# Lainshower/debiasing-multi-modal

Hardware: AMD Instinct MI355X
Metric: images/sec (embed+adapter step), CLIP-RN50 224px bs=1024 (higher is better)
Workload: dtype f32; 1 GPU; CLIP-RN50 224px encode_image + adapter(1024-128-1024) CE/SGD step, 1024 images/GPU, global batch 1024 (the metric's configuration, CLIP-RN50 224px bs=1024 on one GPU); global_batch=1024, batch_per_gpu=1024, parallelism=dp1, collective=none

## Files before the change

### debiasing-multi-modal_amd/csrc/bottleneck_chain.hip

```cpp
#include <stdlib.h>
#include "common.h"

namespace {

struct ChainP {
    const float* a; const float* a_absmax;
    const u16* w3; int w3_exp; const float* sc3; const float* b3;
    const float* res; float* x; float* xp; float* x_absmax;
    const u16* w1; int w1_exp; const float* sc1; const float* b1;
    float* y1; float* y1_absmax;
    int M, N;
    int Ho, Wo;
    const float* a2; const float* a2_absmax; const u16* wd; const float* ratio;
    const u16* w2; int w2_exp; const float* sc2; const float* b2;
    int H, W;
};

template <int RH>
__device__ __forceinline__ int swz(int row) { return RH == 32 ? ((row >> 2) & 3) : (RH == 64 ? ((row >> 1) & 7) : (row & 15)); }

constexpr int BM = 128;

template <int K, int P>
struct ChainGeo {
    static constexpr int BNS = K == 64 ? 64 : 32;
    static constexpr int SLROW = BNS + 4;
    static constexpr int R1_BYTES = BM * SLROW * 4 > 2 * BM * 64 * 2 ? BM * SLROW * 4 : 2 * BM * 64 * 2;
    static constexpr int W3_BYTES = BNS * K * 2;
    static constexpr int W1_BYTES = P * BNS * 2;
    static constexpr int LDS_BYTES = R1_BYTES + W3_BYTES + W1_BYTES;
};

template <int POOL>
__device__ __forceinline__ int row_pixel(const ChainP& p, int m) {
    if constexpr (!POOL) return m;
    const int mp = m >> 2, q = m & 3, wp2 = p.Wo >> 1, hwp = (p.Ho >> 1) * wp2;
    const int n = mp / hwp, rem = mp - n * hwp, hp = rem / wp2;
    return (n * p.Ho + 2 * hp + (q >> 1)) * p.Wo + 2 * (rem - hp * wp2) + (q & 1);
}

constexpr int C2_SROWS = 132, C2_PLANE = C2_SROWS * 32;
constexpr int C2_W2P = 104;
template <int K>
struct Conv2Geo {
    static constexpr int W2_OFF = 2 * C2_PLANE;
    static constexpr int GROUP_BYTES = (2 * C2_PLANE * 2 + K * C2_W2P * 2 + 255) / 256 * 256;
    static constexpr int NST = K == 64 ? 2 : 1;
    static constexpr int Z_OFF = NST * GROUP_BYTES;
    static constexpr int BYTES = Z_OFF + 256;
    static constexpr int STAGE_BYTES = BM * 68 * 4;
};
constexpr int cmax(int a, int b) { return a > b ? a : b; }

template <int K, int P, int POOL, int DUAL = 0, int CONV2 = 0>
__global__ __launch_bounds__(256, 2) void bottleneck_chain_kernel(const ChainP p) {
    static_assert(!DUAL || K == 64, "dual-source variant: layer-1 geometry (K = K2 = 64)");
    static_assert(!CONV2 || !POOL, "the conv2 phase walks pixels in standard order");
    static_assert(K == 64 || K == 128, "conv3 reduction depth: 64 (layer 1) or 128 (layer 2)");
    static_assert(P == 64 || P == 128, "conv1' width");
    using G = ChainGeo<K, P>;
    constexpr int BNS = G::BNS, SLROW = G::SLROW;
    constexpr int KS = K / 16, TN3 = BNS / 32, TN1 = P / 32;
    constexpr int LDS_TOTAL = cmax(G::LDS_BYTES + (DUAL ? BNS * 64 * 2 : 0), CONV2 ? cmax(Conv2Geo<K>::BYTES, Conv2Geo<K>::STAGE_BYTES) : 0);
    __shared__ __attribute__((aligned(256))) unsigned char lds_raw[LDS_TOTAL];
    u16* Ay = (u16*)lds_raw;
    float* slab = (float*)lds_raw;
    u16* W3b = (u16*)(lds_raw + G::R1_BYTES);
    u16* W1b = (u16*)(lds_raw + G::R1_BYTES + G::W3_BYTES);
    u16* Wdb = (u16*)(lds_raw + G::R1_BYTES + G::W3_BYTES + G::W1_BYTES);

    const int tid = threadIdx.x, lane = tid & 63, wave = tid >> 6;
    const int fr = lane & 31, fh = lane >> 5;
    const int m0 = xcd_remap(blockIdx.x, gridDim.x) * BM;
    const int NT = p.N / BNS;

    const int g0 = row_pixel<POOL>(p, m0);
    const long long Mll = p.M;
    const __amdgpu_buffer_rsrc_t rsA = desc(p.a, Mll * K * 4, (long long)g0 * K * 4);
    const __amdgpu_buffer_rsrc_t rsR = DUAL ? desc(p.a2, Mll * 64 * 4, (long long)g0 * 64 * 4)
                                            : desc(p.res, Mll * p.N * 4, (long long)g0 * p.N * 4);
    const __amdgpu_buffer_rsrc_t rsX = desc(p.x, POOL == 2 ? 0 : Mll * p.N * 4, (long long)g0 * p.N * 4);
    const __amdgpu_buffer_rsrc_t rsY = desc(p.y1, Mll * P * 4, (long long)g0 * P * 4);
    __amdgpu_buffer_rsrc_t rsXP = rsX;
    if constexpr (POOL) rsXP = desc(p.xp, (Mll >> 2) * p.N * 4, (long long)(m0 >> 2) * p.N * 4);

    unsigned gx[4], gy[4];
#pragma unroll
    for (int t = 0; t < 4; ++t) {
        const int m = m0 + wave * 32 + 8 * t + 4 * fh;
        const int dp = row_pixel<POOL>(p, m) - g0;
        gx[t] = m < p.M ? (unsigned)dp * (unsigned)(p.N * 4) + (unsigned)(fr * 4) : OOR;
        gy[t] = m < p.M ? (unsigned)dp * (unsigned)(P * 4) + (unsigned)(fr * 4) : OOR;
    }
    auto qpix = [&](int q) { return POOL ? (q >> 1) * p.Wo + (q & 1) : q; };

    constexpr int CPR3 = K / 8, RPP3 = 256 / CPR3, W3LD = BNS * CPR3 / 256;
    constexpr int CPR1 = BNS / 8, RPP1 = 256 / CPR1, W1LD = P * CPR1 / 256;
    static_assert(W3LD >= 1 && W1LD >= 1, "weight slabs smaller than one pass of the workgroup");
    const int wc3 = tid % CPR3, wr3 = tid / CPR3, wc1 = tid % CPR1, wr1 = tid / CPR1;
    u32x4 w3r[W3LD], w1r[W1LD], wdr[DUAL ? W3LD : 1];
    auto load_w = [&](int nt) {
#pragma unroll
        for (int j = 0; j < W3LD; ++j) {
            w3r[j] = *(const u32x4*)(p.w3 + (size_t)(nt * BNS + wr3 + RPP3 * j) * K + wc3 * 8);
            if constexpr (DUAL) wdr[j] = *(const u32x4*)(p.wd + (size_t)(nt * BNS + wr3 + RPP3 * j) * 64 + wc3 * 8);
        }
#pragma unroll
        for (int j = 0; j < W1LD; ++j)
            w1r[j] = *(const u32x4*)(p.w1 + (size_t)(wr1 + RPP1 * j) * p.N + nt * BNS + wc1 * 8);
    };
    auto store_w = [&]() {
#pragma unroll
        for (int j = 0; j < W3LD; ++j) {
            const int row = wr3 + RPP3 * j;
            *(u32x4*)(W3b + row * K + ((wc3 ^ swz<K>(row)) << 3)) = w3r[j];
            if constexpr (DUAL) *(u32x4*)(Wdb + row * 64 + ((wc3 ^ swz<64>(row)) << 3)) = wdr[j];
        }
// ... 44 lines not shown
        __syncthreads();
#pragma unroll
        for (int ks = 0; ks < 4; ++ks) {
            const int row = wave * 32 + fr;
            const int off = row * 64 + (((2 * ks + fh) ^ swz<64>(row)) << 3);
            dst[ks][0] = *(const u32x4*)(Ay + off);
            dst[ks][1] = *(const u32x4*)(Ay + BM * 64 + off);
        }
    };
    auto stage_pass = [&](const __amdgpu_buffer_rsrc_t& rs, int ldk, int k0, float sc, u32x4 (*dst)[2]) {
        f32x4 q[8];
        stage_issue(rs, ldk, k0, q);
        stage_finish(q, sc, dst);
    };
    f32x4 q2[(DUAL && CONV2) ? 8 : 1];
    if constexpr (DUAL && CONV2) stage_issue(rsR, 64, 0, q2);
    int s_a;
    if constexpr (!CONV2) {
        s_a = scale_exp(*p.a_absmax);
#pragma unroll
        for (int kp = 0; kp < K / 64; ++kp) stage_pass(rsA, K, kp * 64, pow2f(s_a), af + kp * 4);
    } else {
        using C2 = Conv2Geo<K>;
        constexpr int TN2 = K / 32, NG = (K / 32) * 3, W2LD = (K * 12 + 255) / 256;
        u16* Sp = (u16*)lds_raw;
        constexpr int NST = C2::NST, STH = C2::GROUP_BYTES / 2;
        constexpr int ZLH = C2::Z_OFF / 2;
        if (tid < 16) *(u32x4*)(lds_raw + C2::Z_OFF + tid * 16) = (u32x4){0u, 0u, 0u, 0u};
        const int s_y1 = scale_exp(*p.a_absmax);
        const float y1_sc = pow2f(s_y1);
        const int px0 = m0 - 1 - p.W > 0 ? m0 - 1 - p.W : 0;
        const __amdgpu_buffer_rsrc_t rsS = desc(p.a, Mll * K * 4, (long long)px0 * K * 4);
        const int lc = tid & 7, lr = tid >> 3;
        unsigned s_off[5];
#pragma unroll
        for (int i = 0; i < 5; ++i) {
            const int j = lr + 32 * i;
            s_off[i] = j < 130 ? (unsigned)((m0 - 1 + j - px0) * (K * 4)) + lc * 16u : OOR;
        }
        unsigned fmask = 0;
        {
            const int m = m0 + wave * 32 + fr;
            if (m < p.M) {
                const int hw = p.H * p.W, rem = m - (m / hw) * hw, ho = rem / p.W, wo = rem - ho * p.W;
#pragma unroll
                for (int kh = 0; kh < 3; ++kh)
#pragma unroll
                    for (int kw = 0; kw < 3; ++kw)
                        if (ho + kh - 1 >= 0 && ho + kh - 1 < p.H && wo + kw - 1 >= 0 && wo + kw - 1 < p.W) fmask |= 1u << (kh * 3 + kw);
            }
        }
        f32x4 sq[5];
        u32x4 w2q[W2LD];
        auto load_group = [&](int g) {
            const int sl = g / 3, kh = g - sl * 3;
            const unsigned delta = (unsigned)(((kh - 1) * p.W * K + sl * 32) * 4);
#pragma unroll
            for (int i = 0; i < 5; ++i)
                sq[i] = __builtin_bit_cast(f32x4, __builtin_amdgcn_raw_buffer_load_b128(rsS, s_off[i] == OOR ? OOR : s_off[i] + delta, 0, 0));
#pragma unroll
            for (int i = 0; i < W2LD; ++i) {
                const int idx = tid + 256 * i, row = idx / 12, c = idx - row * 12;
                w2q[i] = idx < K * 12 ? *(const u32x4*)(p.w2 + (size_t)row * (9 * K) + (size_t)g * 96 + c * 8) : (u32x4){0u, 0u, 0u, 0u};
            }
        };
        auto store_group = [&](int st) {
            u16* Sps = Sp + st * STH;
            u16* W2b = Sps + C2::W2_OFF;
#pragma unroll
            for (int i = 0; i < 5; ++i) {
                const int row = lr + 32 * i;
                if (row < 130) {
                    unsigned hp[2], lp[2];
#pragma unroll
                    for (int j = 0; j < 2; ++j) split2h_pair(sq[i][2 * j], sq[i][2 * j + 1], y1_sc, hp[j], lp[j]);
                    const int off = row * 32 + (((lc >> 1) ^ swz<32>(row)) << 3) + ((lc & 1) << 2);
                    *(u32x2*)(Sps + off) = (u32x2){hp[0], hp[1]};
                    *(u32x2*)(Sps + C2_PLANE + off) = (u32x2){lp[0], lp[1]};
                }
            }
#pragma unroll
            for (int i = 0; i < W2LD; ++i) {
                const int idx = tid + 256 * i, row = idx / 12, c = idx - row * 12;
                if (idx < K * 12) *(u32x4*)(W2b + row * C2_W2P + c * 8) = w2q[i];
            }
        };
        f32x16 acc2[TN2];
#pragma unroll
        for (int j = 0; j < TN2; ++j)
#pragma unroll
            for (int r = 0; r < 16; ++r) acc2[j][r] = 0.f;
        auto compute_group = [&](int g, int st) {
            const u16* Sps = Sp + st * STH;
            const u16* W2b = Sps + C2::W2_OFF;
            const int zl = ZLH - st * STH;
            const int kh = g % 3;
#pragma unroll
            for (int kw = 0; kw < 3; ++kw) {
                const bool ok = (fmask >> (kh * 3 + kw)) & 1u;
                const int row = wave * 32 + fr + kw;
#pragma unroll
                for (int ks = 0; ks < 2; ++ks) {
                    const int addr = row * 32 + (((2 * ks + fh) ^ swz<32>(row)) << 3);
                    const int a0 = ok ? addr : zl + (addr & 127), a1 = ok ? addr + C2_PLANE : zl + (addr & 127);
                    const u32x4 ah = *(const u32x4*)(Sps + a0), al = *(const u32x4*)(Sps + a1);
                    u32x4 wf[TN2];
#pragma unroll
                    for (int j = 0; j < TN2; ++j) wf[j] = *(const u32x4*)(W2b + (j * 32 + fr) * C2_W2P + kw * 32 + (2 * ks + fh) * 8);
#pragma unroll
                    for (int j = 0; j < TN2; ++j)
                        acc2[j] = __builtin_amdgcn_mfma_f32_32x32x16_f16(__builtin_bit_cast(f16x8, al), __builtin_bit_cast(f16x8, wf[j]), acc2[j], 0, 0, 0);
#pragma unroll
                    for (int j = 0; j < TN2; ++j)
                        acc2[j] = __builtin_amdgcn_mfma_f32_32x32x16_f16(__builtin_bit_cast(f16x8, ah), __builtin_bit_cast(f16x8, wf[j]), acc2[j], 0, 0, 0);
                }
            }
        };
        load_group(0);
        if constexpr (NST == 2) {
            store_group(0);
            __syncthreads();
            for (int g = 0; g < NG; ++g) {
                if (g + 1 < NG) load_group(g + 1);
                compute_group(g, g & 1);
                if (g + 1 < NG) store_group((g + 1) & 1);
                __syncthreads();
            }
        } else {
            for (int g = 0; g < NG; ++g) {
                store_group(0);
                __syncthreads();
                if (g + 1 < NG) load_group(g + 1);
                compute_group(g, 0);
                __syncthreads();
            }
        }
        const float c2_scale = pow2f(-s_y1 - p.w2_exp);
        float ymax = 0.f;
#pragma unroll
        for (int j = 0; j < TN2; ++j) {
            const float sv = p.sc2[j * 32 + fr] * c2_scale, bv = p.b2[j * 32 + fr];
#pragma unroll
            for (int r = 0; r < 16; ++r) {
                float v = fmaxf(fmaf(acc2[j][r], sv, bv), 0.f);
                if (gx[r >> 2] == OOR) v = 0.f;
                acc2[j][r] = v;
                ymax = fmaxf(ymax, v);
            }
        }
        s_a = scale_exp(wave_max(ymax));
        const float y2_sc = pow2f(s_a);
        float* St = (float*)lds_raw + wave * (32 * 68);
#pragma unroll
        for (int h = 0; h < K / 64; ++h) {
#pragma unroll
            for (int jj = 0; jj < 2; ++jj)
#pragma unroll
                for (int r = 0; r < 16; ++r) St[((r & 3) + 8 * (r >> 2) + 4 * fh) * 68 + jj * 32 + fr] = acc2[2 * h + jj][r];
#pragma unroll
            for (int ks = 0; ks < 4; ++ks) {
                const f32x4 x0 = *(const f32x4*)(St + fr * 68 + 16 * ks + 8 * fh), x1 = *(const f32x4*)(St + fr * 68 + 16 * ks + 8 * fh + 4);
                unsigned hh[4], ll[4];
                split2h_pair(x0[0], x0[1], y2_sc, hh[0], ll[0]); split2h_pair(x0[2], x0[3], y2_sc, hh[1], ll[1]);
                split2h_pair(x1[0], x1[1], y2_sc, hh[2], ll[2]); split2h_pair(x1[2], x1[3], y2_sc, hh[3], ll[3]);
// ... 29 lines not shown
        f32x16 acc3[TN3];
#pragma unroll
        for (int j = 0; j < TN3; ++j)
#pragma unroll
            for (int r = 0; r < 16; ++r) acc3[j][r] = 0.f;
        if constexpr (DUAL) {
#pragma unroll
            for (int ks = 0; ks < 4; ++ks) {
                u32x4 wf[TN3];
#pragma unroll
                for (int j = 0; j < TN3; ++j) {
                    const int row = j * 32 + fr;
                    wf[j] = *(const u32x4*)(Wdb + row * 64 + (((2 * ks + fh) ^ swz<64>(row)) << 3));
                }
#pragma unroll
                for (int pl = 1; pl >= 0; --pl)
#pragma unroll
                    for (int j = 0; j < TN3; ++j)
                        acc3[j] = __builtin_amdgcn_mfma_f32_32x32x16_f16(__builtin_bit_cast(f16x8, af2[ks][pl]),
                                                                         __builtin_bit_cast(f16x8, wf[j]), acc3[j], 0, 0, 0);
            }
#pragma unroll
            for (int j = 0; j < TN3; ++j) {
                const float rt = p.ratio[n0 + j * 32 + fr] * dual_dyn;
#pragma unroll
                for (int r = 0; r < 16; ++r) acc3[j][r] *= rt;
            }
        }
#pragma unroll
        for (int ks = 0; ks < KS; ++ks) {
            u32x4 wf[TN3];
#pragma unroll
            for (int j = 0; j < TN3; ++j) {
                const int row = j * 32 + fr;
                wf[j] = *(const u32x4*)(W3b + row * K + (((2 * ks + fh) ^ swz<K>(row)) << 3));
            }
#pragma unroll
            for (int pl = 1; pl >= 0; --pl)
#pragma unroll
                for (int j = 0; j < TN3; ++j)
                    acc3[j] = __builtin_amdgcn_mfma_f32_32x32x16_f16(__builtin_bit_cast(f16x8, af[ks][pl]),
                                                                     __builtin_bit_cast(f16x8, wf[j]), acc3[j], 0, 0, 0);
        }
        float tmax = 0.f;
#pragma unroll
        for (int j = 0; j < TN3; ++j) {
            const int n = n0 + j * 32 + fr;
            const float sv = p.sc3[n] * acc3_scale, bv = p.b3[n];
#pragma unroll
            for (int r = 0; r < 16; ++r) {
                float v = fmaxf(fmaf(acc3[j][r], sv, bv) + (DUAL ? 0.f : rr[j][r]), 0.f);
                if (gx[r >> 2] == OOR) v = 0.f;
                acc3[j][r] = v;
                tmax = fmaxf(tmax, v);
                if constexpr (POOL != 2)
                    __builtin_amdgcn_raw_buffer_store_b32(__builtin_bit_cast(unsigned, v), rsX, gx[r >> 2],
                                                          (unsigned)((n0 + j * 32) * 4 + qpix(r & 3) * p.N * 4), 0);
                Ls[((r & 3) + 8 * (r >> 2) + 4 * fh) * SLROW + j * 32 + fr] = v;
            }
            if constexpr (POOL) {
#pragma unroll
                for (int t = 0; t < 4; ++t) {
                    const float s = (((acc3[j][4 * t] + acc3[j][4 * t + 1]) + acc3[j][4 * t + 2]) + acc3[j][4 * t + 3]) * 0.25f;
                    const int mp = wave * 8 + 2 * t + fh;
                    const unsigned off = gx[t] != OOR ? (unsigned)mp * (unsigned)(p.N * 4) + (unsigned)(fr * 4) : OOR;
                    __builtin_amdgcn_raw_buffer_store_b32(__builtin_bit_cast(unsigned, s), rsXP, off, (unsigned)((n0 + j * 32) * 4), 0);
                }
            }
        }
        if (nt + 1 < NT) load_res(nt + 1);
        tmax = wave_max(tmax);
        x_amax = fmaxf(x_amax, tmax);
        if (tmax > run_max) {
            run_max = tmax;
            const int s_new = scale_exp(run_max);
            if (s_new != s_cur) {
                const float f = pow2f(s_new - s_cur);
#pragma unroll
                for (int j = 0; j < TN1; ++j)
#pragma unroll
                    for (int r = 0; r < 16; ++r) acc1[j][r] *= f;
                s_cur = s_new;
            }
        }
        const float t_sc = pow2f(s_cur);
#pragma unroll
        for (int ks = 0; ks < BNS / 16; ++ks) {
            const f32x4 x0 = *(const f32x4*)(Ls + fr * SLROW + 16 * ks + 8 * fh);
            const f32x4 x1 = *(const f32x4*)(Ls + fr * SLROW + 16 * ks + 8 * fh + 4);
            unsigned h[4], l[4];
            split2h_pair(x0[0], x0[1], t_sc, h[0], l[0]); split2h_pair(x0[2], x0[3], t_sc, h[1], l[1]);
            split2h_pair(x1[0], x1[1], t_sc, h[2], l[2]); split2h_pair(x1[2], x1[3], t_sc, h[3], l[3]);
            const u32x4 ah = {h[0], h[1], h[2], h[3]}, al = {l[0], l[1], l[2], l[3]};
// ... 2 lines not shown
            for (int j = 0; j < TN1; ++j) {
                const int row = j * 32 + fr;
                wf[j] = *(const u32x4*)(W1b + row * BNS + (((2 * ks + fh) ^ swz<BNS>(row)) << 3));
            }
#pragma unroll
            for (int j = 0; j < TN1; ++j)
                acc1[j] = __builtin_amdgcn_mfma_f32_32x32x16_f16(__builtin_bit_cast(f16x8, al), __builtin_bit_cast(f16x8, wf[j]),
                                                                 acc1[j], 0, 0, 0);
#pragma unroll
            for (int j = 0; j < TN1; ++j)
                acc1[j] = __builtin_amdgcn_mfma_f32_32x32x16_f16(__builtin_bit_cast(f16x8, ah), __builtin_bit_cast(f16x8, wf[j]),
                                                                 acc1[j], 0, 0, 0);
        }
        __syncthreads();
        if (nt + 1 < NT) store_w();
        __syncthreads();
    }

    float y_amax = 0.f;
    const float acc1_scale = pow2f(-s_cur - p.w1_exp);
#pragma unroll
    for (int j = 0; j < TN1; ++j) {
        const int n = j * 32 + fr;
        const float sv = p.sc1[n] * acc1_scale, bv = p.b1[n];
#pragma unroll
        for (int r = 0; r < 16; ++r) {
            const float v = fmaxf(fmaf(acc1[j][r], sv, bv), 0.f);
            __builtin_amdgcn_raw_buffer_store_b32(__builtin_bit_cast(unsigned, v), rsY, gy[r >> 2],
                                                  (unsigned)(j * 32 * 4 + qpix(r & 3) * P * 4), 0);
            if (gy[r >> 2] != OOR) y_amax = fmaxf(y_amax, v);
        }
    }
    y_amax = wave_max(y_amax);
    float* red = (float*)W3b;
    if (lane == 0) { red[wave] = x_amax; red[4 + wave] = y_amax; }
    __syncthreads();
    if (tid == 0) {
        const float xm = fmaxf(fmaxf(red[0], red[1]), fmaxf(red[2], red[3]));
        const float ym = fmaxf(fmaxf(red[4], red[5]), fmaxf(red[6], red[7]));
        if (p.x_absmax && xm > *(volatile const float*)p.x_absmax) atomicMax((unsigned*)p.x_absmax, __float_as_uint(xm));
        if (p.y1_absmax && ym > *(volatile const float*)p.y1_absmax) atomicMax((unsigned*)p.y1_absmax, __float_as_uint(ym));
    }
}

}

int dbmm_chain8_launch(const float* y2, const float* y2_absmax, const void* w3_plane_f16, int w3_exp, const float* scale3,
                       const float* bias3, const float* residual, float* x_out, float* x_absmax, const void* w1_plane_f16, int w1_exp,
                       const float* scale1, const float* bias1, float* y1_out, float* y1_absmax, int64_t M, int64_t N, void* stream);

extern "C" int dbmm_bottleneck_block_chain_x2(const float* y1, const float* y1_absmax, const void* w2_plane_f16, int w2_exp,
                                              const float* scale2, const float* bias2, const void* w3_plane_f16, int w3_exp,
                                              const float* scale3, const float* bias3, const float* residual, const float* a2,
                                              const float* a2_absmax, const void* wd_plane_f16, const float* ratio, float* x_out,
                                              float* x_absmax, const void* w1_plane_f16, int w1_exp, const float* scale1,
                                              const float* bias1, float* y1_out, float* y1_out_absmax, int64_t B, int64_t H,
                                              int64_t W, int64_t K, int64_t N, int64_t P, void* stream) {
    const bool dual = a2 != nullptr;
    if (!y1 || !y1_absmax || !w2_plane_f16 || !scale2 || !bias2 || !w3_plane_f16 || !scale3 || !bias3 || !x_out || !w1_plane_f16 ||
        !scale1 || !bias1 || !y1_out)
        return DBMM_E_ARG;
    if (dual ? (!a2_absmax || !wd_plane_f16 || !ratio || residual) : (!residual || a2_absmax || wd_plane_f16 || ratio)) return DBMM_E_ARG;
    if (B <= 0 || H <= 0 || W <= 0 || K <= 0 || N <= 0 || P <= 0) return DBMM_E_SHAPE;
    const int64_t M = B * H * W;
    if (M > (INT32_MAX >> 1)) return DBMM_E_SHAPE;
    const bool served = dual ? (K == 64 && P == 64) : ((K == 64 && P == 64) || (K == 128 && P == 128));
    if (!served || (N % 64) != 0 || (M & 3)) return DBMM_E_UNSUPPORTED;
    if (w2_exp < -40 || w2_exp > 40 || w3_exp < -40 || w3_exp > 40 || w1_exp < -40 || w1_exp > 40) return DBMM_E_UNSUPPORTED;
    if (!dbmm_aligned16(y1) || !dbmm_aligned16(w2_plane_f16) || !dbmm_aligned16(w3_plane_f16) || !dbmm_aligned16(w1_plane_f16) ||
        !dbmm_aligned16(x_out) || !dbmm_aligned16(y1_out) || (residual && !dbmm_aligned16(residual)) || (a2 && !dbmm_aligned16(a2)) ||
        (wd_plane_f16 && !dbmm_aligned16(wd_plane_f16)))
        return DBMM_E_ALIGN;
    ChainP p{};
    p.a = y1; p.a_absmax = y1_absmax;
    p.w2 = (const u16*)w2_plane_f16; p.w2_exp = w2_exp; p.sc2 = scale2; p.b2 = bias2; p.H = (int)H; p.W = (int)W;
    p.w3 = (const u16*)w3_plane_f16; p.w3_exp = w3_exp; p.sc3 = scale3; p.b3 = bias3;
    p.res = residual; p.a2 = a2; p.a2_absmax = a2_absmax; p.wd = (const u16*)wd_plane_f16; p.ratio = ratio;
    p.x = x_out; p.x_absmax = x_absmax;
    p.w1 = (const u16*)w1_plane_f16; p.w1_exp = w1_exp; p.sc1 = scale1; p.b1 = bias1;
    p.y1 = y1_out; p.y1_absmax = y1_out_absmax;
    p.M = (int)M; p.N = (int)N; p.Ho = (int)H; p.Wo = (int)W;
    const dim3 grid((unsigned)((M + BM - 1) / BM));
    hipStream_t s = (hipStream_t)stream;
    if (dual) hipLaunchKernelGGL((bottleneck_chain_kernel<64, 64, 0, 1, 1>), grid, dim3(256), 0, s, p);
    else if (K == 64) hipLaunchKernelGGL((bottleneck_chain_kernel<64, 64, 0, 0, 1>), grid, dim3(256), 0, s, p);
    else hipLaunchKernelGGL((bottleneck_chain_kernel<128, 128, 0, 0, 1>), grid, dim3(256), 0, s, p);
    DBMM_CHECK_LAUNCH();
    return DBMM_OK;
}

extern "C" int dbmm_bottleneck_chain_dual_x2(const float* y2, const float* y2_absmax, const void* w3_plane_f16, int w3_exp,
                                             const float* scale3, const float* bias, const float* a2, const float* a2_absmax,
                                             const void* wd_plane_f16, const float* ratio, float* x_out, float* x_absmax,
                                             const void* w1_plane_f16, int w1_exp, const float* scale1, const float* bias1,
                                             float* y1_out, float* y1_absmax, int64_t M, int64_t K, int64_t K2, int64_t N,
                                             int64_t P, void* stream) {
    if (!y2 || !y2_absmax || !w3_plane_f16 || !scale3 || !bias || !a2 || !a2_absmax || !wd_plane_f16 || !ratio || !x_out ||
        !w1_plane_f16 || !scale1 || !bias1 || !y1_out)
        return DBMM_E_ARG;
    if (M <= 0 || K <= 0 || K2 <= 0 || N <= 0 || P <= 0 || M > (INT32_MAX >> 1)) return DBMM_E_SHAPE;
    if (K != 64 || K2 != 64 || (N % 64) != 0 || (P != 64 && P != 128) || (M & 3)) return DBMM_E_UNSUPPORTED;
    if (w3_exp < -40 || w3_exp > 40 || w1_exp < -40 || w1_exp > 40) return DBMM_E_UNSUPPORTED;
    if (!dbmm_aligned16(y2) || !dbmm_aligned16(a2) || !dbmm_aligned16(w3_plane_f16) || !dbmm_aligned16(wd_plane_f16) ||
        !dbmm_aligned16(w1_plane_f16) || !dbmm_aligned16(x_out) || !dbmm_aligned16(y1_out))
        return DBMM_E_ALIGN;
    ChainP p{};
    p.a = y2; p.a_absmax = y2_absmax;
    p.w3 = (const u16*)w3_plane_f16; p.w3_exp = w3_exp; p.sc3 = scale3; p.b3 = bias;
    p.a2 = a2; p.a2_absmax = a2_absmax; p.wd = (const u16*)wd_plane_f16; p.ratio = ratio;
    p.x = x_out; p.x_absmax = x_absmax;
    p.w1 = (const u16*)w1_plane_f16; p.w1_exp = w1_exp; p.sc1 = scale1; p.b1 = bias1;
    p.y1 = y1_out; p.y1_absmax = y1_absmax;
    p.M = (int)M; p.N = (int)N; p.Ho = 1; p.Wo = (int)M;
    const dim3 grid((unsigned)((M + BM - 1) / BM));
    hipStream_t s = (hipStream_t)stream;
    if (P == 64) hipLaunchKernelGGL((bottleneck_chain_kernel<64, 64, 0, 1>), grid, dim3(256), 0, s, p);
    else hipLaunchKernelGGL((bottleneck_chain_kernel<64, 128, 0, 1>), grid, dim3(256), 0, s, p);
    DBMM_CHECK_LAUNCH();
    return DBMM_OK;
}

extern "C" int dbmm_bottleneck_chain_x2(const float* y2, const float* y2_absmax, const void* w3_plane_f16, int w3_exp,
                                        const float* scale3, const float* bias3, const float* residual, float* x_out,
                                        float* x_pooled, float* x_absmax, const void* w1_plane_f16, int w1_exp,
                                        const float* scale1, const float* bias1, float* y1_out, float* y1_absmax,
                                        int64_t B, int64_t Ho, int64_t Wo, int64_t K, int64_t N, int64_t P, void* stream) {
    if (!y2 || !y2_absmax || !w3_plane_f16 || !scale3 || !bias3 || !residual || !w1_plane_f16 || !scale1 || !bias1 || !y1_out)
        return DBMM_E_ARG;
    if (!x_out && !x_pooled) return DBMM_E_ARG;
    if (B <= 0 || Ho <= 0 || Wo <= 0 || K <= 0 || N <= 0 || P <= 0) return DBMM_E_SHAPE;
    const int64_t M = B * Ho * Wo;
    if (M > (INT32_MAX >> 1)) return DBMM_E_SHAPE;
    if (M & 3) return DBMM_E_UNSUPPORTED;
    if (K == 256 && P == 256 && !x_pooled && dbmm_opt(OPT_CHAIN8)) {
        if (w3_exp < -40 || w3_exp > 40 || w1_exp < -40 || w1_exp > 40) return DBMM_E_UNSUPPORTED;
        if (!dbmm_aligned16(y2) || !dbmm_aligned16(w3_plane_f16) || !dbmm_aligned16(w1_plane_f16) || !dbmm_aligned16(residual) ||
            !dbmm_aligned16(x_out) || !dbmm_aligned16(y1_out))
            return DBMM_E_ALIGN;
        return dbmm_chain8_launch(y2, y2_absmax, w3_plane_f16, w3_exp, scale3, bias3, residual, x_out, x_absmax, w1_plane_f16, w1_exp,
                                  scale1, bias1, y1_out, y1_absmax, M, N, stream);
    }
    if ((K != 64 && K != 128) || (N % 64) != 0 || (P != 64 && P != 128)) return DBMM_E_UNSUPPORTED;
    if (w3_exp < -40 || w3_exp > 40 || w1_exp < -40 || w1_exp > 40) return DBMM_E_UNSUPPORTED;
    if (x_pooled && ((Ho & 1) || (Wo & 1))) return DBMM_E_UNSUPPORTED;
    if (!dbmm_aligned16(y2) || !dbmm_aligned16(w3_plane_f16) || !dbmm_aligned16(w1_plane_f16) || !dbmm_aligned16(residual) ||
        (x_out && !dbmm_aligned16(x_out)) || !dbmm_aligned16(y1_out) || (x_pooled && !dbmm_aligned16(x_pooled)))
        return DBMM_E_ALIGN;
    ChainP p{};
    p.a = y2; p.a_absmax = y2_absmax;
    p.w3 = (const u16*)w3_plane_f16; p.w3_exp = w3_exp; p.sc3 = scale3; p.b3 = bias3;
    p.res = residual; p.x = x_out; p.xp = x_pooled; p.x_absmax = x_absmax;
    p.w1 = (const u16*)w1_plane_f16; p.w1_exp = w1_exp; p.sc1 = scale1; p.b1 = bias1;
    p.y1 = y1_out; p.y1_absmax = y1_absmax;
    p.M = (int)M; p.N = (int)N; p.Ho = (int)Ho; p.Wo = (int)Wo;
    const dim3 grid((unsigned)((M + BM - 1) / BM));
    hipStream_t s = (hipStream_t)stream;
#define CHAIN_LAUNCH(KK, PP, PL) hipLaunchKernelGGL((bottleneck_chain_kernel<KK, PP, PL>), grid, dim3(256), 0, s, p)
    if (K == 64) {
        if (!x_out)        { if (P == 64) CHAIN_LAUNCH(64, 64, 2); else CHAIN_LAUNCH(64, 128, 2); }
        else if (x_pooled) { if (P == 64) CHAIN_LAUNCH(64, 64, 1); else CHAIN_LAUNCH(64, 128, 1); }
        else               { if (P == 64) CHAIN_LAUNCH(64, 64, 0); else CHAIN_LAUNCH(64, 128, 0); }
    } else {
        if (!x_out)        { if (P == 64) CHAIN_LAUNCH(128, 64, 2); else CHAIN_LAUNCH(128, 128, 2); }
        else if (x_pooled) { if (P == 64) CHAIN_LAUNCH(128, 64, 1); else CHAIN_LAUNCH(128, 128, 1); }
        else               { if (P == 64) CHAIN_LAUNCH(128, 64, 0); else CHAIN_LAUNCH(128, 128, 0); }
// ... 6 lines not shown
```

### debiasing-multi-modal_amd/csrc/conv1x1_res_stream.hip

```cpp
#include <stdlib.h>
#include <type_traits>
#include "common.h"

namespace {

struct ResStreamP {
    const float* a; const float* a_absmax;
    const u16* w; int w_exp; const float* sc; const float* b;
    const float* res; float* y; float* y_absmax;
    int M, N, n_tiles;
    float* yp; int Ho, Wo;
};

template <int POOL>
__device__ __forceinline__ int row_pixel(const ResStreamP& p, int m) {
    if constexpr (!POOL) return m;
    const int mp = m >> 2, q = m & 3, wp2 = p.Wo >> 1, hwp = (p.Ho >> 1) * wp2;
    const int n = mp / hwp, rem = mp - n * hwp, hp = rem / wp2;
    return (n * p.Ho + 2 * hp + (q >> 1)) * p.Wo + 2 * (rem - hp * wp2) + (q & 1);
}

template <int RH>
__device__ __forceinline__ int swz(int row) { return RH == 64 ? ((row >> 1) & 7) : (row & 15); }

constexpr int BM = 128, BNS = 32;

template <int K, int POOL = 0>
__global__ __launch_bounds__(256, 2) void conv1x1_res_stream_kernel(const ResStreamP p) {
    static_assert(K == 256, "reduction depth (K = 128 compiles and is correct, but measured level with the tile kernel at M = 802,816 and 4 % behind it at 200,704: not instantiated)");
    constexpr int KS = K / 16;
    constexpr int AY_BYTES = 2 * BM * 64 * 2, W_BYTES = BNS * K * 2;
    __shared__ __attribute__((aligned(256))) unsigned char lds_raw[AY_BYTES + 2 * W_BYTES];
    u16* Ay = (u16*)lds_raw;
    u16* Wr = (u16*)(lds_raw + AY_BYTES);
    const int tid = threadIdx.x, lane = tid & 63, wave = tid >> 6;
    const int fr = lane & 31, fh = lane >> 5;
    const int NT = p.N / BNS;
    const long long U = (long long)p.n_tiles * NT;
    long long u = U * blockIdx.x / gridDim.x;
    const long long u_end = U * (blockIdx.x + 1) / gridDim.x;
    const int s_a = scale_exp(*p.a_absmax);
    const float a_sc = pow2f(s_a), acc_scale = pow2f(-s_a - p.w_exp);
    const long long Mll = p.M;

    constexpr int CPR = K / 8, RPP = 256 / CPR, WLD = BNS * CPR / 256;
    const int wc = tid % CPR, wr = tid / CPR;
    u32x4 w3r[WLD];
    float y_amax = 0.f;

    while (u < u_end) {
        const int tile = (int)(u / NT), nt0 = (int)(u - (long long)tile * NT);
        const int nt1 = (long long)(NT - nt0) < u_end - u ? NT : nt0 + (int)(u_end - u);
        u += nt1 - nt0;
        const int m0 = tile * BM;
        const int g0 = row_pixel<POOL>(p, m0);
        const __amdgpu_buffer_rsrc_t rsA = desc(p.a, Mll * K * 4, (long long)g0 * K * 4);
        const __amdgpu_buffer_rsrc_t rsR = desc(p.res, Mll * p.N * 4, (long long)g0 * p.N * 4);
        const __amdgpu_buffer_rsrc_t rsY = desc(p.y, Mll * p.N * 4, (long long)g0 * p.N * 4);
        __amdgpu_buffer_rsrc_t rsP = rsY;
        if constexpr (POOL) rsP = desc(p.yp, (Mll >> 2) * p.N * 4, (long long)(m0 >> 2) * p.N * 4);
        unsigned gx[4];
#pragma unroll
        for (int t = 0; t < 4; ++t) {
            const int row = wave * 32 + 8 * t + 4 * fh;
            gx[t] = m0 + row < p.M ? (unsigned)(row_pixel<POOL>(p, m0 + row) - g0) * (unsigned)(p.N * 4) + (unsigned)(fr * 4) : OOR;
        }
        auto qpix = [&](int q) { return POOL ? (q >> 1) * p.Wo + (q & 1) : q; };
        auto load_w = [&](int nt) {
#pragma unroll
            for (int j = 0; j < WLD; ++j) w3r[j] = *(const u32x4*)(p.w + (size_t)(nt * BNS + wr + RPP * j) * K + wc * 8);
        };
        auto store_w = [&](int slot) {
#pragma unroll
            for (int j = 0; j < WLD; ++j) {
                const int row = wr + RPP * j;
                *(u32x4*)(Wr + slot * (BNS * K) + row * K + ((wc ^ swz<K>(row)) << 3)) = w3r[j];
            }
        };
        float rr[2][16];
        auto load_res = [&](int nt, auto slot_c) {
            constexpr int S = decltype(slot_c)::value;
#pragma unroll
            for (int r = 0; r < 16; ++r)
                rr[S][r] = __builtin_bit_cast(float, __builtin_amdgcn_raw_buffer_load_b32(rsR, gx[r >> 2], (unsigned)((nt * BNS) * 4 + qpix(r & 3) * p.N * 4), 0));
        };
        load_w(nt0);
        load_res(nt0, std::integral_constant<int, 0>());
        u32x4 af[KS][2];
        {
            const int lc = tid & 15, lr = tid >> 4;
#pragma unroll
            for (int kp = 0; kp < K / 64; ++kp) {
                f32x4 q[8];
#pragma unroll
                for (int i = 0; i < 8; ++i) {
                    const int row = lr + 16 * i;
                    const unsigned off = m0 + row < p.M ? (unsigned)(row_pixel<POOL>(p, m0 + row) - g0) * (unsigned)(K * 4) + lc * 16u : OOR;
                    q[i] = __builtin_bit_cast(f32x4, __builtin_amdgcn_raw_buffer_load_b128(rsA, off, (unsigned)(kp * 64 * 4), 0));
                }
                __syncthreads();
#pragma unroll
                for (int i = 0; i < 8; ++i) {
                    const int row = lr + 16 * i;
                    unsigned hp[2], lp[2];
#pragma unroll
                    for (int j = 0; j < 2; ++j) split2h_pair(q[i][2 * j], q[i][2 * j + 1], a_sc, hp[j], lp[j]);
                    const int off = row * 64 + (((lc >> 1) ^ swz<64>(row)) << 3) + ((lc & 1) << 2);
                    *(u32x2*)(Ay + off) = (u32x2){hp[0], hp[1]};
                    *(u32x2*)(Ay + BM * 64 + off) = (u32x2){lp[0], lp[1]};
                }
                if (kp == 0) store_w(0);
                __syncthreads();
#pragma unroll
                for (int ks = 0; ks < 4; ++ks) {
                    const int row = wave * 32 + fr;
                    const int off = row * 64 + (((2 * ks + fh) ^ swz<64>(row)) << 3);
                    af[4 * kp + ks][0] = *(const u32x4*)(Ay + off);
                    af[4 * kp + ks][1] = *(const u32x4*)(Ay + BM * 64 + off);
                }
            }
        }
        if (nt0 + 1 < nt1) load_res(nt0 + 1, std::integral_constant<int, 1>());
        auto slab = [&](int nt, auto slot_c) {
            constexpr int S = decltype(slot_c)::value;
            if (nt + 1 < nt1) load_w(nt + 1);
            f32x16 acc;
#pragma unroll
            for (int r = 0; r < 16; ++r) acc[r] = 0.f;
            const u16* Wb = Wr + S * (BNS * K);
#pragma unroll
            for (int ks = 0; ks < KS; ++ks) {
                const u32x4 wf = *(const u32x4*)(Wb + fr * K + (((2 * ks + fh) ^ swz<K>(fr)) << 3));
                acc = __builtin_amdgcn_mfma_f32_32x32x16_f16(__builtin_bit_cast(f16x8, af[ks][1]), __builtin_bit_cast(f16x8, wf), acc, 0, 0, 0);
                acc = __builtin_amdgcn_mfma_f32_32x32x16_f16(__builtin_bit_cast(f16x8, af[ks][0]), __builtin_bit_cast(f16x8, wf), acc, 0, 0, 0);
            }
            const int n = nt * BNS + fr;
            const float sv = p.sc[n] * acc_scale, bv = p.b ? p.b[n] : 0.f;
#pragma unroll
            for (int r = 0; r < 16; ++r) {
                const float v = fmaxf(fmaf(acc[r], sv, bv) + rr[S][r], 0.f);
                acc[r] = v;
                __builtin_amdgcn_raw_buffer_store_b32(__builtin_bit_cast(unsigned, v), rsY, gx[r >> 2], (unsigned)((nt * BNS) * 4 + qpix(r & 3) * p.N * 4), 0);
                if (gx[r >> 2] != OOR) y_amax = fmaxf(y_amax, v);
            }
            if constexpr (POOL) {
#pragma unroll
                for (int t = 0; t < 4; ++t) {
                    const float sm = (((acc[4 * t] + acc[4 * t + 1]) + acc[4 * t + 2]) + acc[4 * t + 3]) * 0.25f;
                    const int mp = wave * 8 + 2 * t + fh;
                    __builtin_amdgcn_raw_buffer_store_b32(__builtin_bit_cast(unsigned, sm), rsP,
                                                          gx[t] != OOR ? (unsigned)mp * (unsigned)(p.N * 4) + (unsigned)(fr * 4) : OOR, (unsigned)((nt * BNS) * 4), 0);
                }
            }
            if (nt + 2 < nt1) load_res(nt + 2, slot_c);
            if (nt + 1 < nt1) store_w(S ^ 1);
            __syncthreads();
        };
        for (int nt = nt0; nt < nt1; nt += 2) {
            slab(nt, std::integral_constant<int, 0>());
            if (nt + 1 < nt1) slab(nt + 1, std::integral_constant<int, 1>());
        }
    }
    if (p.y_absmax) {
        y_amax = wave_max(y_amax);
        float* red = (float*)lds_raw;
        if (lane == 0) red[wave] = y_amax;
        __syncthreads();
        if (tid == 0) {
            const float m = fmaxf(fmaxf(red[0], red[1]), fmaxf(red[2], red[3]));
            if (m > *(volatile const float*)p.y_absmax) atomicMax((unsigned*)p.y_absmax, __float_as_uint(m));
        }
    }
}

}

int dbmm_conv1x1_res_stream(const float* a, const float* a_absmax, const void* w_plane_f16, int w_exp, const float* scale, const float* bias,
                            const float* residual, float* y, float* y_pooled, float* y_absmax, int64_t M, int64_t Ho, int64_t Wo, int64_t K,
                            int64_t N, void* stream) {
    if (!a || !a_absmax || !w_plane_f16 || !scale || !residual || !y) return DBMM_E_ARG;
    if (M <= 0 || N <= 0 || M > (INT32_MAX >> 1)) return DBMM_E_SHAPE;
    if (K != 256 || (N % BNS) || (M & 3) || w_exp < -40 || w_exp > 40) return DBMM_E_UNSUPPORTED;
    if (y_pooled && (Ho <= 0 || Wo <= 0 || (Ho & 1) || (Wo & 1) || M % (Ho * Wo))) return DBMM_E_UNSUPPORTED;
    if ((132LL + (y_pooled ? 2 * Wo : 0)) * N * 4 >= EXT_LIM) return DBMM_E_UNSUPPORTED;
    if (!dbmm_aligned16(a) || !dbmm_aligned16(w_plane_f16) || !dbmm_aligned16(residual) || !dbmm_aligned16(y) || (y_pooled && !dbmm_aligned16(y_pooled)))
        return DBMM_E_ALIGN;
    ResStreamP p{};
    p.a = a; p.a_absmax = a_absmax; p.w = (const u16*)w_plane_f16; p.w_exp = w_exp; p.sc = scale; p.b = bias; p.res = residual; p.y = y;
    p.y_absmax = y_absmax; p.M = (int)M; p.N = (int)N; p.n_tiles = (int)((M + BM - 1) / BM);
    p.yp = y_pooled; p.Ho = (int)Ho; p.Wo = (int)Wo;
    const long long units = (long long)p.n_tiles * (N / BNS);
    const int grid = (int)(units < 2 * DBMM_N_CU ? units : 2 * DBMM_N_CU);
    hipStream_t s = (hipStream_t)stream;
    if (y_pooled) hipLaunchKernelGGL((conv1x1_res_stream_kernel<256, 1>), dim3(grid), dim3(256), 0, s, p);
    else hipLaunchKernelGGL((conv1x1_res_stream_kernel<256, 0>), dim3(grid), dim3(256), 0, s, p);
    DBMM_CHECK_LAUNCH();
    return DBMM_OK;
}
```

Baseline: 36930 images/sec.

## Stage per-channel scale/bias in LDS and make chain/stream loads unconditional

Per-channel scale, bias and ratio vectors are copied into LDS at kernel start with buffer-load-to-LDS, and epilogues read them from LDS instead of global memory. The conv2 phase gets double register sets with a two-group unrolled prefetch loop, and its W2 and residual prefetch loads become unconditional buffer loads that use a zero-size descriptor instead of branches, so the compiler's wait counts are less conservative. Residual prefetch for the next slab is moved earlier in one variant. The cost is more LDS per block, which may lower occupancy, plus more registers from the doubled prefetch sets, and new N<=NMAX limits.

```diff
diff --git a/debiasing-multi-modal_amd/csrc/bottleneck_chain.hip b/debiasing-multi-modal_amd/csrc/bottleneck_chain.hip
--- a/debiasing-multi-modal_amd/csrc/bottleneck_chain.hip
+++ b/debiasing-multi-modal_amd/csrc/bottleneck_chain.hip
@@ -1,4 +1,5 @@
 #include <stdlib.h>
+#include <type_traits>
 #include "common.h"
 
 namespace {
@@ -20,6 +21,15 @@
 __device__ __forceinline__ int swz(int row) { return RH == 32 ? ((row >> 2) & 3) : (RH == 64 ? ((row >> 1) & 7) : (row & 15)); }
 
 constexpr int BM = 128;
+constexpr int NMAX = 1024;
+
+__device__ __forceinline__ void glds4(__amdgpu_buffer_rsrc_t r, unsigned char* lds_dst, unsigned voff) {
+#if defined(__HIP_DEVICE_COMPILE__)
+    __builtin_amdgcn_raw_ptr_buffer_load_lds(r, (__attribute__((address_space(3))) void*)lds_dst, 4, voff, 0, 0, 0);
+#else
+    (void)r; (void)lds_dst; (void)voff;
+#endif
+}
 
 template <int K, int P>
 struct ChainGeo {
@@ -61,8 +71,16 @@
     using G = ChainGeo<K, P>;
     constexpr int BNS = G::BNS, SLROW = G::SLROW;
     constexpr int KS = K / 16, TN3 = BNS / 32, TN1 = P / 32;
-    constexpr int LDS_TOTAL = cmax(G::LDS_BYTES + (DUAL ? BNS * 64 * 2 : 0), CONV2 ? cmax(Conv2Geo<K>::BYTES, Conv2Geo<K>::STAGE_BYTES) : 0);
+    constexpr int LDS_MAIN = (cmax(G::LDS_BYTES + (DUAL ? BNS * 64 * 2 : 0), CONV2 ? cmax(Conv2Geo<K>::BYTES, Conv2Geo<K>::STAGE_BYTES) : 0) + 255) / 256 * 256;
+    constexpr int LDS_TOTAL = LDS_MAIN + ((DUAL ? 3 : 2) * NMAX + 2 * 128 + (CONV2 ? 2 * 128 : 0)) * 4;
     __shared__ __attribute__((aligned(256))) unsigned char lds_raw[LDS_TOTAL];
+    float* V3s = (float*)(lds_raw + LDS_MAIN);
+    float* V3b = V3s + NMAX;
+    float* Vrt = V3b + NMAX;
+    float* V1s = V3b + (DUAL ? 2 : 1) * NMAX;
+    float* V1b = V1s + 128;
+    float* V2s = V1b + 128;
+    float* V2b = V2s + 128;
     u16* Ay = (u16*)lds_raw;
     float* slab = (float*)lds_raw;
     u16* W3b = (u16*)(lds_raw + G::R1_BYTES);
@@ -81,6 +99,7 @@
                                             : desc(p.res, Mll * p.N * 4, (long long)g0 * p.N * 4);
     const __amdgpu_buffer_rsrc_t rsX = desc(p.x, POOL == 2 ? 0 : Mll * p.N * 4, (long long)g0 * p.N * 4);
     const __amdgpu_buffer_rsrc_t rsY = desc(p.y1, Mll * P * 4, (long long)g0 * P * 4);
+    const __amdgpu_buffer_rsrc_t rsZ = desc(p.a, 0, 0);
     __amdgpu_buffer_rsrc_t rsXP = rsX;
     if constexpr (POOL) rsXP = desc(p.xp, (Mll >> 2) * p.N * 4, (long long)(m0 >> 2) * p.N * 4);
 
@@ -93,6 +112,25 @@
         gy[t] = m < p.M ? (unsigned)dp * (unsigned)(P * 4) + (unsigned)(fr * 4) : OOR;
     }
     auto qpix = [&](int q) { return POOL ? (q >> 1) * p.Wo + (q & 1) : q; };
+
+    {
+        const unsigned vo = (unsigned)tid * 4u;
+        const __amdgpu_buffer_rsrc_t rs3s = desc(p.sc3, (long long)p.N * 4, 0), rs3b = desc(p.b3, (long long)p.N * 4, 0);
+#pragma unroll
+        for (int j = 0; j < NMAX / 256; ++j) {
+            glds4(rs3s, (unsigned char*)(V3s + 256 * j + 64 * wave), vo + 1024u * j);
+            glds4(rs3b, (unsigned char*)(V3b + 256 * j + 64 * wave), vo + 1024u * j);
+            if constexpr (DUAL) glds4(desc(p.ratio, (long long)p.N * 4, 0), (unsigned char*)(Vrt + 256 * j + 64 * wave), vo + 1024u * j);
+        }
+        if (wave < 2) {
+            glds4(desc(p.sc1, P * 4, 0), (unsigned char*)(V1s + 64 * wave), vo);
+            glds4(desc(p.b1, P * 4, 0), (unsigned char*)(V1b + 64 * wave), vo);
+            if constexpr (CONV2) {
+                glds4(desc(p.sc2, K * 4, 0), (unsigned char*)(V2s + 64 * wave), vo);
+                glds4(desc(p.b2, K * 4, 0), (unsigned char*)(V2b + 64 * wave), vo);
+            }
+        }
+    }
 
     constexpr int CPR3 = K / 8, RPP3 = 256 / CPR3, W3LD = BNS * CPR3 / 256;
     constexpr int CPR1 = BNS / 8, RPP1 = 256 / CPR1, W1LD = P * CPR1 / 256;
@@ -183,7 +221,8 @@
         for (int kp = 0; kp < K / 64; ++kp) stage_pass(rsA, K, kp * 64, pow2f(s_a), af + kp * 4);
     } else {
         using C2 = Conv2Geo<K>;
-        constexpr int TN2 = K / 32, NG = (K / 32) * 3, W2LD = (K * 12 + 255) / 256;
+        constexpr int TN2 = K / 32, NG = (K / 32) * 3, W2LD = K * 12 / 256;
+        static_assert(K * 12 % 256 == 0, "a W2 group is whole passes of the workgroup: its loads carry no condition (a branch around a load makes the compiler's wait counts conservative)");
         u16* Sp = (u16*)lds_raw;
         constexpr int NST = C2::NST, STH = C2::GROUP_BYTES / 2;
         constexpr int ZLH = C2::Z_OFF / 2;
@@ -211,21 +250,32 @@
                         if (ho + kh - 1 >= 0 && ho + kh - 1 < p.H && wo + kw - 1 >= 0 && wo + kw - 1 < p.W) fmask |= 1u << (kh * 3 + kw);
             }
         }
-        f32x4 sq[5];
-        u32x4 w2q[W2LD];
-        auto load_group = [&](int g) {
+        constexpr int NSET = K == 64 ? 2 : 1;
+        f32x4 sq_[NSET][5];
+        u32x4 w2q_[NSET][W2LD];
+        const __amdgpu_buffer_rsrc_t rsW2 = desc(p.w2, (long long)K * 9 * K * 2, 0);
+        unsigned w2_off[W2LD];
+#pragma unroll
+        for (int i = 0; i < W2LD; ++i) {
+            const int idx = tid + 256 * i, row = idx / 12, c = idx - row * 12;
+            w2_off[i] = (unsigned)(row * (9 * K) + c * 8) * 2u;
+        }
+        auto load_group = [&](int g, auto set_c) {
+            f32x4 (&sq)[5] = sq_[decltype(set_c)::value];
+            u32x4 (&w2q)[W2LD] = w2q_[decltype(set_c)::value];
             const int sl = g / 3, kh = g - sl * 3;
             const unsigned delta = (unsigned)(((kh - 1) * p.W * K + sl * 32) * 4);
+            const __amdgpu_buffer_rsrc_t rs = g < NG ? rsS : rsZ, rw = g < NG ? rsW2 : rsZ;
 #pragma unroll
             for (int i = 0; i < 5; ++i)
-                sq[i] = __builtin_bit_cast(f32x4, __builtin_amdgcn_raw_buffer_load_b128(rsS, s_off[i] == OOR ? OOR : s_off[i] + delta, 0, 0));
-#pragma unroll
-            for (int i = 0; i < W2LD; ++i) {
-                const int idx = tid + 256 * i, row = idx / 12, c = idx - row * 12;
-                w2q[i] = idx < K * 12 ? *(const u32x4*)(p.w2 + (size_t)row * (9 * K) + (size_t)g * 96 + c * 8) : (u32x4){0u, 0u, 0u, 0u};
-            }
+                sq[i] = __builtin_bit_cast(f32x4, __builtin_amdgcn_raw_buffer_load_b128(rs, s_off[i] == OOR ? OOR : s_off[i] + delta, 0, 0));
+#pragma unroll
+            for (int i = 0; i < W2LD; ++i)
+                w2q[i] = __builtin_bit_cast(u32x4, __builtin_amdgcn_raw_buffer_load_b128(rw, w2_off[i], (unsigned)(g * 96 * 2), 0));
         };
-        auto store_group = [&](int st) {
+        auto store_group = [&](int st, auto set_c) {
+            const f32x4 (&sq)[5] = sq_[decltype(set_c)::value];
+            const u32x4 (&w2q)[W2LD] = w2q_[decltype(set_c)::value];
             u16* Sps = Sp + st * STH;
             u16* W2b = Sps + C2::W2_OFF;
 #pragma unroll
@@ -243,7 +293,7 @@
 #pragma unroll
             for (int i = 0; i < W2LD; ++i) {
                 const int idx = tid + 256 * i, row = idx / 12, c = idx - row * 12;
-                if (idx < K * 12) *(u32x4*)(W2b + row * C2_W2P + c * 8) = w2q[i];
+                *(u32x4*)(W2b + row * C2_W2P + c * 8) = w2q[i];
             }
         };
         f32x16 acc2[TN2];
@@ -277,21 +327,30 @@
                 }
             }
         };
-        load_group(0);
+        constexpr std::integral_constant<int, 0> set0{};
+        constexpr std::integral_constant<int, NSET - 1> set1{};
+        load_group(0, set0);
         if constexpr (NST == 2) {
-            store_group(0);
+            static_assert(NSET == 2 && NG % 2 == 0, "the group loop is unrolled by the two register sets");
+            load_group(1, set1);
+            store_group(0, set0);
+            load_group(2, set0);
             __syncthreads();
-            for (int g = 0; g < NG; ++g) {
-                if (g + 1 < NG) load_group(g + 1);
-                compute_group(g, g & 1);
-                if (g + 1 < NG) store_group((g + 1) & 1);
+            for (int g = 0; g < NG; g += 2) {
+                compute_group(g, 0);
+                store_group(1, set1);
+                load_group(g + 3, set1);
+                __syncthreads();
+                compute_group(g + 1, 1);
+                if (g + 2 < NG) store_group(0, set0);
+                load_group(g + 4, set0);
                 __syncthreads();
             }
         } else {
             for (int g = 0; g < NG; ++g) {
-                store_group(0);
+                store_group(0, set0);
                 __syncthreads();
-                if (g + 1 < NG) load_group(g + 1);
+                load_group(g + 1, set0);
                 compute_group(g, 0);
                 __syncthreads();
             }
@@ -300,7 +359,7 @@
         float ymax = 0.f;
 #pragma unroll
         for (int j = 0; j < TN2; ++j) {
-            const float sv = p.sc2[j * 32 + fr] * c2_scale, bv = p.b2[j * 32 + fr];
+            const float sv = V2s[j * 32 + fr] * c2_scale, bv = V2b[j * 32 + fr];
 #pragma unroll
             for (int r = 0; r < 16; ++r) {
                 float v = fmaxf(fmaf(acc2[j][r], sv, bv), 0.f);
@@ -376,7 +435,7 @@
             }
 #pragma unroll
             for (int j = 0; j < TN3; ++j) {
-                const float rt = p.ratio[n0 + j * 32 + fr] * dual_dyn;
+                const float rt = Vrt[n0 + j * 32 + fr] * dual_dyn;
 #pragma unroll
                 for (int r = 0; r < 16; ++r) acc3[j][r] *= rt;
             }
@@ -400,13 +459,25 @@
 #pragma unroll
         for (int j = 0; j < TN3; ++j) {
             const int n = n0 + j * 32 + fr;
-            const float sv = p.sc3[n] * acc3_scale, bv = p.b3[n];
+            const float sv = V3s[n] * acc3_scale, bv = V3b[n];
 #pragma unroll
             for (int r = 0; r < 16; ++r) {
                 float v = fmaxf(fmaf(acc3[j][r], sv, bv) + (DUAL ? 0.f : rr[j][r]), 0.f);
                 if (gx[r >> 2] == OOR) v = 0.f;
                 acc3[j][r] = v;
                 tmax = fmaxf(tmax, v);
+            }
+        }
+        constexpr bool RES_EARLY = !DUAL && POOL == 2;
+        const __amdgpu_buffer_rsrc_t rsRn = nt + 1 < NT ? rsR : rsZ;
+#pragma unroll
+        for (int j = 0; j < TN3; ++j) {
+#pragma unroll
+            for (int r = 0; r < 16; ++r) {
+                const float v = acc3[j][r];
+                if constexpr (RES_EARLY)
+                    rr[j][r] = __builtin_bit_cast(float, __builtin_amdgcn_raw_buffer_load_b32(
+                        rsRn, gx[r >> 2], (unsigned)((n0 + BNS + j * 32) * 4 + qpix(r & 3) * p.N * 4), 0));
                 if constexpr (POOL != 2)
                     __builtin_amdgcn_raw_buffer_store_b32(__builtin_bit_cast(unsigned, v), rsX, gx[r >> 2],
                                                           (unsigned)((n0 + j * 32) * 4 + qpix(r & 3) * p.N * 4), 0);
@@ -422,7 +493,14 @@
                 }
             }
         }
-        if (nt + 1 < NT) load_res(nt + 1);
+        if constexpr (!DUAL && !RES_EARLY) {
+#pragma unroll
+            for (int j = 0; j < TN3; ++j)
+#pragma unroll
+                for (int r = 0; r < 16; ++r)
+                    rr[j][r] = __builtin_bit_cast(float, __builtin_amdgcn_raw_buffer_load_b32(
+                        rsRn, gx[r >> 2], (unsigned)((n0 + BNS + j * 32) * 4 + qpix(r & 3) * p.N * 4), 0));
+        }
         tmax = wave_max(tmax);
         x_amax = fmaxf(x_amax, tmax);
         if (tmax > run_max) {
@@ -471,7 +549,7 @@
 #pragma unroll
     for (int j = 0; j < TN1; ++j) {
         const int n = j * 32 + fr;
-        const float sv = p.sc1[n] * acc1_scale, bv = p.b1[n];
+        const float sv = V1s[n] * acc1_scale, bv = V1b[n];
 #pragma unroll
         for (int r = 0; r < 16; ++r) {
             const float v = fmaxf(fmaf(acc1[j][r], sv, bv), 0.f);
@@ -514,7 +592,7 @@
     const int64_t M = B * H * W;
     if (M > (INT32_MAX >> 1)) return DBMM_E_SHAPE;
     const bool served = dual ? (K == 64 && P == 64) : ((K == 64 && P == 64) || (K == 128 && P == 128));
-    if (!served || (N % 64) != 0 || (M & 3)) return DBMM_E_UNSUPPORTED;
+    if (!served || (N % 64) != 0 || N > NMAX || (M & 3)) return DBMM_E_UNSUPPORTED;
     if (w2_exp < -40 || w2_exp > 40 || w3_exp < -40 || w3_exp > 40 || w1_exp < -40 || w1_exp > 40) return DBMM_E_UNSUPPORTED;
     if (!dbmm_aligned16(y1) || !dbmm_aligned16(w2_plane_f16) || !dbmm_aligned16(w3_plane_f16) || !dbmm_aligned16(w1_plane_f16) ||
         !dbmm_aligned16(x_out) || !dbmm_aligned16(y1_out) || (residual && !dbmm_aligned16(residual)) || (a2 && !dbmm_aligned16(a2)) ||
@@ -548,7 +626,7 @@
         !w1_plane_f16 || !scale1 || !bias1 || !y1_out)
         return DBMM_E_ARG;
     if (M <= 0 || K <= 0 || K2 <= 0 || N <= 0 || P <= 0 || M > (INT32_MAX >> 1)) return DBMM_E_SHAPE;
-    if (K != 64 || K2 != 64 || (N % 64) != 0 || (P != 64 && P != 128) || (M & 3)) return DBMM_E_UNSUPPORTED;
+    if (K != 64 || K2 != 64 || (N % 64) != 0 || N > NMAX || (P != 64 && P != 128) || (M & 3)) return DBMM_E_UNSUPPORTED;
     if (w3_exp < -40 || w3_exp > 40 || w1_exp < -40 || w1_exp > 40) return DBMM_E_UNSUPPORTED;
     if (!dbmm_aligned16(y2) || !dbmm_aligned16(a2) || !dbmm_aligned16(w3_plane_f16) || !dbmm_aligned16(wd_plane_f16) ||
         !dbmm_aligned16(w1_plane_f16) || !dbmm_aligned16(x_out) || !dbmm_aligned16(y1_out))
@@ -589,7 +667,7 @@
         return dbmm_chain8_launch(y2, y2_absmax, w3_plane_f16, w3_exp, scale3, bias3, residual, x_out, x_absmax, w1_plane_f16, w1_exp,
                                   scale1, bias1, y1_out, y1_absmax, M, N, stream);
     }
-    if ((K != 64 && K != 128) || (N % 64) != 0 || (P != 64 && P != 128)) return DBMM_E_UNSUPPORTED;
+    if ((K != 64 && K != 128) || (N % (K == 64 ? 64 : 32)) != 0 || N > NMAX || (P != 64 && P != 128)) return DBMM_E_UNSUPPORTED;
     if (w3_exp < -40 || w3_exp > 40 || w1_exp < -40 || w1_exp > 40) return DBMM_E_UNSUPPORTED;
     if (x_pooled && ((Ho & 1) || (Wo & 1))) return DBMM_E_UNSUPPORTED;
     if (!dbmm_aligned16(y2) || !dbmm_aligned16(w3_plane_f16) || !dbmm_aligned16(w1_plane_f16) || !dbmm_aligned16(residual) ||
diff --git a/debiasing-multi-modal_amd/csrc/conv1x1_res_stream.hip b/debiasing-multi-modal_amd/csrc/conv1x1_res_stream.hip
--- a/debiasing-multi-modal_amd/csrc/conv1x1_res_stream.hip
+++ b/debiasing-multi-modal_amd/csrc/conv1x1_res_stream.hip
@@ -25,14 +25,25 @@
 
 constexpr int BM = 128, BNS = 32;
 
+__device__ __forceinline__ void glds4(__amdgpu_buffer_rsrc_t r, unsigned char* lds_dst, unsigned voff) {
+#if defined(__HIP_DEVICE_COMPILE__)
+    __builtin_amdgcn_raw_ptr_buffer_load_lds(r, (__attribute__((address_space(3))) void*)lds_dst, 4, voff, 0, 0, 0);
+#else
+    (void)r; (void)lds_dst; (void)voff;
+#endif
+}
+constexpr int NMAX = 2048;
+
 template <int K, int POOL = 0>
 __global__ __launch_bounds__(256, 2) void conv1x1_res_stream_kernel(const ResStreamP p) {
     static_assert(K == 256, "reduction depth (K = 128 compiles and is correct, but measured level with the tile kernel at M = 802,816 and 4 % behind it at 200,704: not instantiated)");
     constexpr int KS = K / 16;
     constexpr int AY_BYTES = 2 * BM * 64 * 2, W_BYTES = BNS * K * 2;
-    __shared__ __attribute__((aligned(256))) unsigned char lds_raw[AY_BYTES + 2 * W_BYTES];
+    __shared__ __attribute__((aligned(256))) unsigned char lds_raw[AY_BYTES + 2 * W_BYTES + 2 * NMAX * 4];
     u16* Ay = (u16*)lds_raw;
     u16* Wr = (u16*)(lds_raw + AY_BYTES);
+    float* Vs = (float*)(lds_raw + AY_BYTES + 2 * W_BYTES);
+    float* Vb = Vs + NMAX;
     const int tid = threadIdx.x, lane = tid & 63, wave = tid >> 6;
     const int fr = lane & 31, fh = lane >> 5;
     const int NT = p.N / BNS;
@@ -48,22 +59,35 @@
     u32x4 w3r[WLD];
     float y_amax = 0.f;
 
+    {
+        const __amdgpu_buffer_rsrc_t rsS = desc(p.sc, (long long)p.N * 4, 0), rsB = desc(p.b ? p.b : p.sc, p.b ? (long long)p.N * 4 : 0, 0);
+#pragma unroll
+        for (int j = 0; j < NMAX / 256; ++j) {
+            glds4(rsS, (unsigned char*)(Vs + 256 * j + 64 * wave), (unsigned)(256 * j + tid) * 4u);
+            glds4(rsB, (unsigned char*)(Vb + 256 * j + 64 * wave), (unsigned)(256 * j + tid) * 4u);
+        }
+    }
+
     while (u < u_end) {
         const int tile = (int)(u / NT), nt0 = (int)(u - (long long)tile * NT);
         const int nt1 = (long long)(NT - nt0) < u_end - u ? NT : nt0 + (int)(u_end - u);
         u += nt1 - nt0;
         const int m0 = tile * BM;
+        int tseg = tid;
+        asm volatile("" : "+v"(tseg));
+        const int wave_s = tseg >> 6, fr_s = tseg & 31, fh_s = (tseg >> 5) & 1;
         const int g0 = row_pixel<POOL>(p, m0);
         const __amdgpu_buffer_rsrc_t rsA = desc(p.a, Mll * K * 4, (long long)g0 * K * 4);
         const __amdgpu_buffer_rsrc_t rsR = desc(p.res, Mll * p.N * 4, (long long)g0 * p.N * 4);
         const __amdgpu_buffer_rsrc_t rsY = desc(p.y, Mll * p.N * 4, (long long)g0 * p.N * 4);
+        const __amdgpu_buffer_rsrc_t rsZ = desc(p.res, 0, 0);
         __amdgpu_buffer_rsrc_t rsP = rsY;
         if constexpr (POOL) rsP = desc(p.yp, (Mll >> 2) * p.N * 4, (long long)(m0 >> 2) * p.N * 4);
         unsigned gx[4];
 #pragma unroll
         for (int t = 0; t < 4; ++t) {
-            const int row = wave * 32 + 8 * t + 4 * fh;
-            gx[t] = m0 + row < p.M ? (unsigned)(row_pixel<POOL>(p, m0 + row) - g0) * (unsigned)(p.N * 4) + (unsigned)(fr * 4) : OOR;
+            const int row = wave_s * 32 + 8 * t + 4 * fh_s;
+            gx[t] = m0 + row < p.M ? (unsigned)(row_pixel<POOL>(p, m0 + row) - g0) * (unsigned)(p.N * 4) + (unsigned)(fr_s * 4) : OOR;
         }
         auto qpix = [&](int q) { return POOL ? (q >> 1) * p.Wo + (q & 1) : q; };
         auto load_w = [&](int nt) {
@@ -88,7 +112,7 @@
         load_res(nt0, std::integral_constant<int, 0>());
         u32x4 af[KS][2];
         {
-            const int lc = tid & 15, lr = tid >> 4;
+            const int lc = tseg & 15, lr = tseg >> 4;
 #pragma unroll
             for (int kp = 0; kp < K / 64; ++kp) {
                 f32x4 q[8];
@@ -113,8 +137,8 @@
                 __syncthreads();
 #pragma unroll
                 for (int ks = 0; ks < 4; ++ks) {
-                    const int row = wave * 32 + fr;
-                    const int off = row * 64 + (((2 * ks + fh) ^ swz<64>(row)) << 3);
+                    const int row = wave_s * 32 + fr_s;
+                    const int off = row * 64 + (((2 * ks + fh_s) ^ swz<64>(row)) << 3);
                     af[4 * kp + ks][0] = *(const u32x4*)(Ay + off);
                     af[4 * kp + ks][1] = *(const u32x4*)(Ay + BM * 64 + off);
                 }
@@ -135,7 +159,8 @@
                 acc = __builtin_amdgcn_mfma_f32_32x32x16_f16(__builtin_bit_cast(f16x8, af[ks][0]), __builtin_bit_cast(f16x8, wf), acc, 0, 0, 0);
             }
             const int n = nt * BNS + fr;
-            const float sv = p.sc[n] * acc_scale, bv = p.b ? p.b[n] : 0.f;
+            const float sv = Vs[n] * acc_scale, bv = Vb[n];
+            const __amdgpu_buffer_rsrc_t rsN = nt + 2 < nt1 ? rsR : rsZ;
 #pragma unroll
             for (int r = 0; r < 16; ++r) {
                 const float v = fmaxf(fmaf(acc[r], sv, bv) + rr[S][r], 0.f);
@@ -152,7 +177,9 @@
                                                           gx[t] != OOR ? (unsigned)mp * (unsigned)(p.N * 4) + (unsigned)(fr * 4) : OOR, (unsigned)((nt * BNS) * 4), 0);
                 }
             }
-            if (nt + 2 < nt1) load_res(nt + 2, slot_c);
+#pragma unroll
+            for (int r = 0; r < 16; ++r)
+                rr[S][r] = __builtin_bit_cast(float, __builtin_amdgcn_raw_buffer_load_b32(rsN, gx[r >> 2], (unsigned)(((nt + 2) * BNS) * 4 + qpix(r & 3) * p.N * 4), 0));
             if (nt + 1 < nt1) store_w(S ^ 1);
             __syncthreads();
         };
@@ -180,7 +207,7 @@
                             int64_t N, void* stream) {
     if (!a || !a_absmax || !w_plane_f16 || !scale || !residual || !y) return DBMM_E_ARG;
     if (M <= 0 || N <= 0 || M > (INT32_MAX >> 1)) return DBMM_E_SHAPE;
-    if (K != 256 || (N % BNS) || (M & 3) || w_exp < -40 || w_exp > 40) return DBMM_E_UNSUPPORTED;
+    if (K != 256 || (N % BNS) || N > NMAX || (M & 3) || w_exp < -40 || w_exp > 40) return DBMM_E_UNSUPPORTED;
     if (y_pooled && (Ho <= 0 || Wo <= 0 || (Ho & 1) || (Wo & 1) || M % (Ho * Wo))) return DBMM_E_UNSUPPORTED;
     if ((132LL + (y_pooled ? 2 * Wo : 0)) * N * 4 >= EXT_LIM) return DBMM_E_UNSUPPORTED;
     if (!dbmm_aligned16(a) || !dbmm_aligned16(w_plane_f16) || !dbmm_aligned16(residual) || !dbmm_aligned16(y) || (y_pooled && !dbmm_aligned16(y_pooled)))
```

Measured after the change: 37250 images/sec, median of 6. Within noise of the previous version (+0.9%).
